# wvu-navLab/corenav-GP

Measured on AMD Instinct MI355X. Metric: GP-fits/s, higher is better.
Workload: dtype f64; 1 GPU; BASELINE configs[1]: batch of independent fixed-theta GP fits, N=2048 d=6 M=599 kernel=SE-ARD f64; streams=0, pipeline_depth=1, N=2048, d=6, M=599, inputs=resident in HBM, ranks=1

## Files before the change

corenav_gp_amd/csrc/cgp_kernels_fused.hpp:

```cpp
#pragma once
#include "cgp_kernels.hpp"

namespace cgp {

#ifndef CGP_SKIP_DEAD_WAVE
#define CGP_SKIP_DEAD_WAVE 1
#endif
constexpr bool kSkipDeadWave = CGP_SKIP_DEAD_WAVE != 0;

template <typename T>
__device__ __forceinline__ void stage_first_chunk(const T *gR, size_t ldR, const T *gC, size_t ldC, T *smem, int tid) {
  constexpr int CH = KT * LDST;
  if constexpr (sizeof(T) == 8) {
    typedef __attribute__((address_space(3))) void lds_void;
    typedef const __attribute__((address_space(1))) void gbl_void;
    const int lane = tid & 63;
    const int wave = __builtin_amdgcn_readfirstlane(tid >> 6);
#pragma unroll
    for (int i = 0; i < KT / 4; ++i) {
      const int col = wave * (KT / 4) + i;
      __builtin_amdgcn_global_load_lds((gbl_void *)(gR + (size_t)col * ldR + lane * 2), (lds_void *)(smem + col * LDST), 16, 0, 0);
      __builtin_amdgcn_global_load_lds((gbl_void *)(gC + (size_t)col * ldC + lane * 2), (lds_void *)(smem + CH + col * LDST), 16, 0, 0);
    }
  } else {
// ... 365 lines not shown
constexpr int BXP_NBUF = 3;
struct BxPlaneSrc {
  const unsigned short *gR, *gC;
  size_t chunk_stride, plane_stride;
  __device__ __forceinline__ void init(const unsigned short *planes, size_t plane_elems, int ld, int chunk0, int row_tile, int col_tile, int tid) {
    const int lane = tid & 63, wave = __builtin_amdgcn_readfirstlane(tid >> 6);
    const int slot = 32 * wave + (lane >> 1);
    const int h = ((lane & 1) ^ (slot >> 2) ^ (slot >> 4)) & 1;
    const int rowR = (slot & ~31) | ((slot & 15) << 1) | ((slot >> 4) & 1);
    chunk_stride = (size_t)ld * BXS;
    plane_stride = plane_elems;
    const unsigned short *base = planes + (size_t)chunk0 * chunk_stride;
    gR = base + ((size_t)row_tile * TS + rowR) * BXS + 8 * h;
    gC = base + ((size_t)col_tile * TS + slot) * BXS + 8 * h;
  }
  __device__ __forceinline__ void issue(int c, unsigned char *smem_bytes, int buf, int wave) const {
    typedef __attribute__((address_space(3))) void lds_void;
    typedef const __attribute__((address_space(1))) void gbl_void;
    const unsigned short *r = gR + (size_t)c * chunk_stride, *q = gC + (size_t)c * chunk_stride;
    unsigned char *dst = smem_bytes + buf + wave * 1024;
#pragma unroll
    for (int pl = 0; pl < 3; ++pl) {
      __builtin_amdgcn_global_load_lds((gbl_void *)(r + pl * plane_stride), (lds_void *)(dst + pl * 2 * BX_PLANE), 16, 0, 0);
      __builtin_amdgcn_global_load_lds((gbl_void *)(q + pl * plane_stride), (lds_void *)(dst + (3 + pl) * 2 * BX_PLANE), 16, 0, 0);
    }
  }
};
__device__ __forceinline__ void store_tile_planes(const Prec<float>::acc_t (&acc)[NCB][2], unsigned short *planes, size_t plane_elems, int ld, int rt, int k,
                                                  int tid) {
  const int lane = tid & 63, l15 = lane & 15, lq = lane >> 4;
  const int wave = __builtin_amdgcn_readfirstlane(tid >> 6);
  typedef unsigned bxu2 __attribute__((ext_vector_type(2)));
  unsigned short *out = planes + ((size_t)(k * (TS / KT)) * ld + (size_t)rt * TS + wave * 32 + 2 * l15) * BXS + 4 * lq;
#pragma unroll
  for (int cb = 0; cb < NCB; ++cb) {
    const float v[8] = {acc[cb][0][0], acc[cb][0][1], acc[cb][0][2], acc[cb][0][3], acc[cb][1][0], acc[cb][1][1], acc[cb][1][2], acc[cb][1][3]};
    bxu4 w[3];
    bx_split8(v, w);
    unsigned short *o = out + (size_t)cb * ld * BXS;
#pragma unroll
    for (int pl = 0; pl < 3; ++pl) {
      *reinterpret_cast<bxu2 *>(o + pl * plane_elems) = bxu2{w[pl][0], w[pl][1]};
      *reinterpret_cast<bxu2 *>(o + pl * plane_elems + BXS) = bxu2{w[pl][2], w[pl][3]};
    }
  }
}
__device__ __forceinline__ void bx6p_loop(Prec<float>::acc_t (&acc)[NCB][2], const BxPlaneSrc &src, int nchunk, float *smem, int tid, const float *zs, float *ms,
                                          bool live, const float *gR32, size_t ldR32) {
  if (nchunk <= 0) return;
  unsigned char *sb = reinterpret_cast<unsigned char *>(smem);
  const int lane = tid & 63, l15 = lane & 15, lq = lane >> 4;
  const int wave = __builtin_amdgcn_readfirstlane(tid >> 6);
  const int hi = lq >> 1;
  const unsigned base = (unsigned)(size_t)smem;
  const unsigned lb0[2] = {base + 2 * bx_pos(wave * 32 + l15, lq & 1), base + 2 * bx_pos(wave * 32 + DB + l15, lq & 1)};
  const unsigned la0[2] = {base + 2 * (3 * BX_PLANE + bx_pos(l15, lq & 1)), base + 2 * (3 * BX_PLANE + bx_pos(DB + l15, lq & 1) - DB * BXS)};
  int buf = 0;
  for (int c = 0; c < nchunk; ++c) {
    asm volatile("s_waitcnt vmcnt(6)" ::: "memory");
    lds_barrier();
    const int nb = buf == 0 ? 2 * BXP_BUF : buf - BXP_BUF;
    src.issue(c + 2 < nchunk ? c + 2 : nchunk - 1, sb, nb, wave);
    if (live) {
      const unsigned la[2] = {la0[0] + buf, la0[1] + buf}, lb[2] = {lb0[0] + buf, lb0[1] + buf};
      bx6_compute_pipe<0>(acc, la, lb, hi);
    }
    buf = buf == 2 * BXP_BUF ? 0 : buf + BXP_BUF;
  }
  asm volatile("s_waitcnt vmcnt(0)" ::: "memory");
  __syncthreads();
  if (zs) {
    const int r = tid & (TS - 1), h8 = 8 * (tid >> 7), zfirst = nchunk - TS / KT;
    float pz = 0.f, pv = 0.f;
    const float *g = gR32 + (size_t)(zfirst * KT + h8) * ldR32 + r;
#pragma unroll
    for (int c = 0; c < TS / KT; ++c) {
      float x[8];
#pragma unroll
      for (int i = 0; i < 8; ++i) x[i] = g[(size_t)(c * KT + i) * ldR32];
#pragma unroll
      for (int i = 0; i < 8; ++i) {
        pz = __builtin_fmaf(x[i], zs[c * KT + h8 + i], pz);
        pv = __builtin_fmaf(x[i], x[i], pv);
      }
    }
    smem[tid] = pz;
    smem[2 * TS + tid] = pv;
    __syncthreads();
    if (lane < 16) {
#pragma unroll
      for (int j = 0; j < 2; ++j) {
        const int rr = wave * 32 + 2 * lane + j;
        ms[j] = smem[rr] + smem[TS + rr];
        ms[2 + j] = smem[2 * TS + rr] + smem[3 * TS + rr];
      }
    }
    __syncthreads();
  }
}

template <typename T, int R = 4> struct RowFrag {
  using vec2 = T __attribute__((ext_vector_type(2)));
  vec2 r[R][KT / 4];
};
#ifndef CGP_MID_RING
#define CGP_MID_RING 4
#endif
template <typename T, bool MID> constexpr int deep_ring() { return (MID && sizeof(T) == 4) ? CGP_MID_RING : 4; }
template <int R> constexpr int deep_dist() { return R == 4 ? 2 : 5; }

template <typename T, int SLOT, int R>
__device__ __forceinline__ void rfrag_load(RowFrag<T, R> &f, const T *gRl, size_t ldR, int chunk, int lq) {
#pragma unroll
  for (int ks = 0; ks < KT / 4; ++ks) {
    const T *src = gRl + (size_t)(chunk * KT + ks * 4 + lq) * ldR;
    if constexpr (sizeof(T) == 8) asm volatile("global_load_dwordx4 %0, %1, off" : "=&v"(f.r[SLOT][ks]) : "v"(src));
    else asm volatile("global_load_dwordx2 %0, %1, off" : "=&v"(f.r[SLOT][ks]) : "v"(src));
  }
}

template <typename T> constexpr int cpanel_loads() { return sizeof(T) == 8 ? KT / 4 : KT / 2; }
template <typename T>
__device__ __forceinline__ void cpanel_stage(const T *gC, size_t ldC, int chunk, T *buf, int lane, int wave) {
  typedef __attribute__((address_space(3))) void lds_void;
  typedef const __attribute__((address_space(1))) void gbl_void;
#pragma unroll
  for (int i = 0; i < KT / 4; ++i) {
    const int col = wave * (KT / 4) + i;
    const T *src = gC + (size_t)(chunk * KT + col) * ldC;
    if constexpr (sizeof(T) == 8) {
      __builtin_amdgcn_global_load_lds((gbl_void *)(src + lane * 2), (lds_void *)(buf + col * LDST), 16, 0, 0);
    } else {
      __builtin_amdgcn_global_load_lds((gbl_void *)(src + lane), (lds_void *)(buf + col * LDST), 4, 0, 0);
      __builtin_amdgcn_global_load_lds((gbl_void *)(src + 64 + lane), (lds_void *)(buf + col * LDST + 64), 4, 0, 0);
    }
  }
}

template <typename T, int R = 4>
__device__ __forceinline__ void rdirect_prologue(RowFrag<T, R> &f, const T *gR, size_t ldR, const T *gC, size_t ldC,
                                                 int nchunk, T *smem, int tid) {
  constexpr int CH = KT * LDST;
  if (nchunk <= 0) return;
  const int lane = tid & 63;
  const int wave = __builtin_amdgcn_readfirstlane(tid >> 6);
  const T *gRl = gR + wave * 32 + 2 * (lane & 15);
  static_for<0, deep_dist<R>()>([&](auto jc) {
    constexpr int J = decltype(jc)::value;
    cpanel_stage<T>(gC, ldC, J, smem + J * CH, lane, wave);
    rfrag_load<T, J>(f, gRl, ldR, J, lane >> 4);
  });
}

template <typename T, int R, int S, bool ISSUE, int WAITN, bool ACC = false>
__device__ __forceinline__ void rdirect_step(typename Prec<T>::acc_t (&acc)[NCB][2], RowFrag<T, R> &f, const T *gRl, size_t ldR,
                                             const T *gC, size_t ldC, int c, T *smem, int lane, int wave,
                                             const T *zs = nullptr, T *ms = nullptr) {
  using P = Prec<T>;
  constexpr int CH = KT * LDST;
  constexpr int D = deep_dist<R>();
  const int l15 = lane & 15, lq = lane >> 4;
  static_assert(WAITN >= 0 && WAITN <= 63, "vmcnt is a 6-bit counter");
  asm volatile("s_waitcnt vmcnt(%0)\n\ts_barrier" ::"n"(WAITN) : "memory");
#pragma unroll
  for (int ks = 0; ks < KT / 4; ++ks) asm volatile("" : "+v"(f.r[S][ks]));
  if constexpr (ISSUE) {
    cpanel_stage<T>(gC, ldC, c + D, smem + ((S + D) % R) * CH, lane, wave);
    rfrag_load<T, (S + D) % R>(f, gRl, ldR, c + D, lq);
  }
  const T *cur = smem + S * CH + lq * LDST + l15;
  T fa[2][NCB];
#pragma unroll
  for (int cb = 0; cb < NCB; ++cb) fa[0][cb] = cur[cb * DB];
#pragma unroll
  for (int ks = 0; ks < KT / 4; ++ks) {
    if (ks + 1 < KT / 4) {
#pragma unroll
      for (int cb = 0; cb < NCB; ++cb) fa[(ks + 1) & 1][cb] = cur[(ks + 1) * 4 * LDST + cb * DB];
    }
    const typename RowFrag<T, R>::vec2 fb = f.r[S][ks];
    if constexpr (ACC) {
      const T zv = zs[ks * 4 + lq];
      ms[0] = __builtin_fma(fb[0], zv, ms[0]);
      ms[1] = __builtin_fma(fb[1], zv, ms[1]);
      ms[2] = __builtin_fma(fb[0], fb[0], ms[2]);
      ms[3] = __builtin_fma(fb[1], fb[1], ms[3]);
    }
#pragma unroll
    for (int cb = 0; cb < NCB; ++cb) {
      acc[cb][0] = P::mfma(fa[ks & 1][cb], fb[0], acc[cb][0]);
      acc[cb][1] = P::mfma(fa[ks & 1][cb], fb[1], acc[cb][1]);
    }
  }
}

template <typename T, int R = 4>
__device__ __forceinline__ void mfma_rowpanel_loop_rdirect(typename Prec<T>::acc_t (&acc)[NCB][2], RowFrag<T, R> &f, const T *gR,
                                                           size_t ldR, const T *gC, size_t ldC, int nchunk, T *smem, int tid,
                                                           const T *zs, T (&ms)[4]) {
  if (nchunk <= 0) return;
  constexpr int D = deep_dist<R>();
  constexpr int L = cpanel_loads<T>() + KT / 4;
  static_assert((D - 1) * L <= 63 && D < R && 8 % R == 0, "ring / distance / vmcnt");
  const int lane = tid & 63;
  const int wave = __builtin_amdgcn_readfirstlane(tid >> 6);
  const T *gRl = gR + wave * 32 + 2 * (lane & 15);
  int c = 0;
  for (; c + 8 < nchunk; c += R) {
    static_for<0, R>([&](auto jc) {
      constexpr int J = decltype(jc)::value;
      rdirect_step<T, R, J, true, (D - 1) * L>(acc, f, gRl, ldR, gC, ldC, c + J, smem, lane, wave);
    });
  }
  static_for<0, 8>([&](auto jc) {
    constexpr int J = decltype(jc)::value;
    constexpr int behind = (D - 1) < (7 - J) ? (D - 1) : (7 - J);
    rdirect_step<T, R, J % R, (J + D < 8), behind * L, true>(acc, f, gRl, ldR, gC, ldC, c + J, smem, lane, wave, zs + J * KT, ms);
  });
}

constexpr int TRI_PD = 2;
__device__ __forceinline__ constexpr int tri_buf(int i) { return i * KT * LDST; }

template <typename T> constexpr int tri_dma_loads() { return sizeof(T) == 8 ? KT / 4 : KT / 2; }
template <typename T, bool DEEP = sizeof(T) == 8>
__device__ __forceinline__ void stage_chunk_tri(const T *gR, size_t ldR, int chunk, T *buf, int tid) {
  if constexpr (DEEP) {
    typedef __attribute__((address_space(3))) void lds_void;
    typedef const __attribute__((address_space(1))) void gbl_void;
    const int lane = tid & 63;
    const int wave = __builtin_amdgcn_readfirstlane(tid >> 6);
#pragma unroll
    for (int i = 0; i < KT / 4; ++i) {
      const int col = wave * (KT / 4) + i;
      const T *src = gR + (size_t)(chunk * KT + col) * ldR;
      if constexpr (sizeof(T) == 8) {
        __builtin_amdgcn_global_load_lds((gbl_void *)(src + lane * 2), (lds_void *)(buf + col * LDST), 16, 0, 0);
      } else {
        __builtin_amdgcn_global_load_lds((gbl_void *)(src + lane), (lds_void *)(buf + col * LDST), 4, 0, 0);
        __builtin_amdgcn_global_load_lds((gbl_void *)(src + 64 + lane), (lds_void *)(buf + col * LDST + 64), 4, 0, 0);
      }
    }
  } else {
    using vec8 = T __attribute__((ext_vector_type(8)));
    const int sc = tid >> 4, sr = (tid & 15) * 8;
    *reinterpret_cast<vec8 *>(buf + sc * LDST + sr) = *reinterpret_cast<const vec8 *>(gR + sr + (size_t)(chunk * KT + sc) * ldR);
  }
}

template <typename T, int W, bool DEEP>
__device__ __forceinline__ void syrk_tri_wave(typename Prec<T>::acc_t (&acc)[NCB][2], const T *gR, size_t ldR, int nchunk,
                                              T *smem, int tid) {
  using P = Prec<T>;
  constexpr int RB0 = W, RB1 = NCB - 1 - W;
  const int lane = tid & 63;
  const int l15 = lane & 15, lq = lane >> 4;

  auto compute = [&](const T *cur) {
#pragma unroll
    for (int ks = 0; ks < KT / 4; ++ks) {
      const T *ra = cur + (ks * 4 + lq) * LDST + l15;
      T fa[RB1 + 1];
#pragma unroll
      for (int cb = 0; cb <= RB1; ++cb) fa[cb] = ra[cb * DB];
#pragma unroll
      for (int cb = 0; cb <= RB1; ++cb) {
        if (cb <= RB0) acc[cb][0] = P::mfma(fa[cb], fa[RB0], acc[cb][0]);
        acc[cb][1] = P::mfma(fa[cb], fa[RB1], acc[cb][1]);
      }
    }
  };

  if constexpr (DEEP) {
    for (int c = 0; c < nchunk; ++c) {
      if (c + 1 < nchunk) {
        if constexpr (sizeof(T) == 8) asm volatile("s_waitcnt vmcnt(4)\n\ts_barrier" ::: "memory");
        else asm volatile("s_waitcnt vmcnt(8)\n\ts_barrier" ::: "memory");
      } else asm volatile("s_waitcnt vmcnt(0)\n\ts_barrier" ::: "memory");
      static_assert(tri_dma_loads<double>() == 4 && tri_dma_loads<float>() == 8, "vmcnt constants");
      if (c + TRI_PD < nchunk) stage_chunk_tri<T, true>(gR, ldR, c + TRI_PD, smem + tri_buf((c + TRI_PD) % (TRI_PD + 1)), tid);
      compute(smem + tri_buf(c % (TRI_PD + 1)));
    }
  } else {
    using vec8 = T __attribute__((ext_vector_type(8)));
    const int sc = tid >> 4, sr = (tid & 15) * 8;
    const T *src = gR + sr + (size_t)sc * ldR;
    __syncthreads();
    for (int c = 0; c < nchunk; ++c) {
      vec8 pr;
      if (c + 1 < nchunk) pr = *reinterpret_cast<const vec8 *>(src + (size_t)((c + 1) * KT) * ldR);
      compute(smem + tri_buf(c & 1));
      if (c + 1 < nchunk) *reinterpret_cast<vec8 *>(smem + tri_buf((c + 1) & 1) + sc * LDST + sr) = pr;
      __syncthreads();
    }
  }
}

template <typename T, bool DEEP = sizeof(T) == 8>
__device__ __forceinline__ void mfma_syrk_tri_loop(typename Prec<T>::acc_t (&acc)[NCB][2], const T *gR, size_t ldR,
                                                   int nchunk, T *smem, int tid) {
  const int wave = __builtin_amdgcn_readfirstlane(tid >> 6);
  switch (wave) {
    case 0: syrk_tri_wave<T, 0, DEEP>(acc, gR, ldR, nchunk, smem, tid); break;
    case 1: syrk_tri_wave<T, 1, DEEP>(acc, gR, ldR, nchunk, smem, tid); break;
    case 2: syrk_tri_wave<T, 2, DEEP>(acc, gR, ldR, nchunk, smem, tid); break;
    default: syrk_tri_wave<T, 3, DEEP>(acc, gR, ldR, nchunk, smem, tid); break;
  }
}
template <typename T, bool DEEP = sizeof(T) == 8>
__device__ __forceinline__ void tri_prologue(const T *gR, size_t ldR, int nchunk, T *smem, int tid) {
  if (nchunk > 0) stage_chunk_tri<T, DEEP>(gR, ldR, 0, smem + tri_buf(0), tid);
  if (DEEP && nchunk > 1) stage_chunk_tri<T, DEEP>(gR, ldR, 1, smem + tri_buf(1), tid);
}

constexpr int BXT_FLOATS = 3 * BX_PLANE / 2;
template <int D> struct BxTriStage {
  __amdgpu_buffer_rsrc_t rR;
  int ldR4, vR, offR;
  float xr[D][8];
  __device__ __forceinline__ void init(const float *gR, size_t ldR, int nchunk, int tid) {
    const int r = tid & (TS - 1), h = tid >> 7;
    rR = __builtin_amdgcn_make_buffer_rsrc(const_cast<float *>(gR), 0, (int)(((size_t)(nchunk > 0 ? nchunk : 0) * KT * ldR) * sizeof(float)), 0x00020000);
    ldR4 = (int)ldR * 4;
    vR = 4 * r + 8 * h * ldR4;
    offR = bx_pos(r, h);
  }
  template <int S> __device__ __forceinline__ void load(int chunk) {
#pragma unroll
    for (int i = 0; i < 8; ++i) xr[S][i] = __builtin_bit_cast(float, __builtin_amdgcn_raw_buffer_load_b32(rR, vR, (chunk * KT + i) * ldR4, 0));
  }
  template <int S> __device__ __forceinline__ void store(float *planes) { bx_split_store(xr[S], reinterpret_cast<unsigned short *>(planes), offR); }
};
template <int D> __device__ __forceinline__ void bx6_tri_prologue(BxTriStage<D> &st) {
  static_assert(D == 2 || D == 4, "register sets (the plane buffer of a chunk follows the parity of its set)");
  st.template load<0>(0);
  st.template load<1>(1);
  if (D > 2) st.template load<2 % D>(2);
  if (D > 2) st.template load<3 % D>(3);
}
template <int W, int BO>
__device__ __forceinline__ void bx6_tri_compute(Prec<float>::acc_t (&acc)[NCB][2], const unsigned (&e)[2], bool hi) {
  constexpr int RB0 = W, RB1 = NCB - 1 - W, PB = 2 * BX_PLANE, CBB = 2 * DB * BXS;
  const unsigned o02 = hi ? 2 * PB : 0, o01 = hi ? PB : 0, o20 = hi ? 0 : 2 * PB, o10 = hi ? 0 : PB;
  bxu4 a02[RB1 + 1], a01[RB1 + 1];
  bxu4 b20[2] = {bx_rd(e[RB0 & 1] + o20, BO + RB0 * CBB), bx_rd(e[RB1 & 1] + o20, BO + RB1 * CBB)};
  static_for<0, RB1 + 1>([&](auto cc) {
    constexpr int CB = decltype(cc)::value;
    a02[CB] = bx_rd(e[CB & 1] + o02, BO + CB * CBB);
  });
  bxu4 b10[2] = {bx_rd(e[RB0 & 1] + o10, BO + RB0 * CBB), bx_rd(e[RB1 & 1] + o10, BO + RB1 * CBB)};
  asm volatile("s_waitcnt lgkmcnt(2)" : "+v"(b20[0]), "+v"(b20[1]));
  static_for<0, RB1 + 1>([&](auto cc) { bx_tie(a02[decltype(cc)::value]); });
  static_for<0, RB1 + 1>([&](auto cc) {
    constexpr int CB = decltype(cc)::value;
    a01[CB] = bx_rd(e[CB & 1] + o01, BO + CB * CBB);
  });
  const bf8 c20[2] = {__builtin_bit_cast(bf8, b20[0]), __builtin_bit_cast(bf8, b20[1])};
  static_for<0, RB1 + 1>([&](auto cc) {
    constexpr int CB = decltype(cc)::value;
    const bf8 a = __builtin_bit_cast(bf8, a02[CB]);
    if constexpr (CB <= RB0) acc[CB][0] = __builtin_amdgcn_mfma_f32_16x16x32_bf16(a, c20[0], acc[CB][0], 0, 0, 0);
    acc[CB][1] = __builtin_amdgcn_mfma_f32_16x16x32_bf16(a, c20[1], acc[CB][1], 0, 0, 0);
  });
  asm volatile("s_waitcnt lgkmcnt(0)" : "+v"(b10[0]), "+v"(b10[1]));
  static_for<0, RB1 + 1>([&](auto cc) { bx_tie(a01[decltype(cc)::value]); });
  const bf8 c10[2] = {__builtin_bit_cast(bf8, b10[0]), __builtin_bit_cast(bf8, b10[1])};
  const bf8 c01[2] = {__builtin_bit_cast(bf8, a01[RB0]), __builtin_bit_cast(bf8, a01[RB1])};
  static_for<0, RB1 + 1>([&](auto cc) {
    constexpr int CB = decltype(cc)::value;
    const bf8 a = __builtin_bit_cast(bf8, a01[CB]);
// ... 387 lines not shown
  if (tid == 0 && bad != 0 && p.info[b] == 0) p.info[b] = bad;
  for (int idx = tid; idx < 28 * DB * DB; idx += 256) {
    const int blk = idx >> 8, e = idx & 255;
    int i = 1, rem = blk;
    while (rem >= i) {
      rem -= i;
      ++i;
    }
    const int j = rem, c = e >> 4, r = e & 15;
    Wk[wimg_blk(i, j) + c * DB + r] = -Bk[tri_blk(i, j) + r * DB + c];
  }
}

enum { DIAG_FULL = 0, DIAG_PARTIAL = 1, DIAG_FINISH = 2 };
__device__ __forceinline__ int img_slots(const FitArgs &p) { return p.img_slots > 0 ? p.img_slots : 2; }
constexpr bool kTriDiag = true;
constexpr int DPART = 2 * NCB * 4 * 256;

template <typename T, bool TRI, bool STORE>
__device__ __forceinline__ void acc_image(typename Prec<T>::acc_t (&acc)[NCB][2], T *__restrict__ img, int tid) {
  const int wave = __builtin_amdgcn_readfirstlane(tid >> 6);
#pragma unroll
  for (int cb = 0; cb < NCB; ++cb)
#pragma unroll
    for (int j = 0; j < 2; ++j) {
      if (TRI && cb > (j ? NCB - 1 - wave : wave)) continue;
#pragma unroll
      for (int r = 0; r < 4; ++r) {
        T *q = img + ((cb * 2 + j) * 4 + r) * 256 + tid;
        if constexpr (STORE) *q = acc[cb][j][r];
        else acc[cb][j][r] = *q;
      }
    }
}

template <typename T> constexpr int potf2_lds_elems() { return TS * LDP + 8 * DB * DB + 4 * DB * DB + 8; }
template <typename T, int MODE, bool TRI, bool DEEP = sizeof(T) == 8, bool FAT = false, bool MAT = false>
__device__ __forceinline__ void diag_next(const FitArgs &p, typename Prec<T>::acc_t (&acc)[NCB][2], T *__restrict__ smem,
                                          T *__restrict__ Lw, int b, int kn, int tid, PhaseClock *pc = nullptr, bool img_ready = false) {
  using P = Prec<T>;
  using vec2 = T __attribute__((ext_vector_type(2)));
  const int ld = p.ld;
  const int lane = tid & 63;
  const int wave = __builtin_amdgcn_readfirstlane(tid >> 6);
  const int l15 = lane & 15;
  constexpr int CH2 = 2 * KT * LDST;
  if constexpr (MODE == DIAG_FINISH) {
    __builtin_amdgcn_fence(__ATOMIC_RELEASE, "workgroup");
    __syncthreads();
    __builtin_amdgcn_fence(__ATOMIC_ACQUIRE, "workgroup");
  }
  const bool from_image = MODE == DIAG_FINISH && kn >= 3;
  const int c_first = from_image ? (kn - 2) * (TS / KT) : 0;
  const int c_last = (MODE == DIAG_PARTIAL ? kn - 2 : kn) * (TS / KT);
  const int nchunk = c_last - c_first;
  const T *gR = Lw + (size_t)kn * TS + (size_t)c_first * KT * ld;
  T *img = reinterpret_cast<T *>(p.dpart) + ((size_t)b * img_slots(p) + kn % img_slots(p)) * DPART;
  constexpr bool BXT = kF32Bf16x6 && kBxTri && sizeof(T) == 4 && TRI && DEEP;
  BxTriStage<kBxMidSets> bxt;
  {
    GramPre<T> gp;
    if (!from_image) gram_prefetch<T>(p, b, kn, kn, tid, gp);
    if constexpr (BXT) {
      bxt.init(gR, (size_t)ld, nchunk, tid);
      bx6_tri_prologue(bxt);
    } else if constexpr (TRI) tri_prologue<T, DEEP>(gR, (size_t)ld, nchunk, smem, tid);
    else if (nchunk > 0) stage_first_chunk<T>(gR, (size_t)ld, gR, (size_t)ld, smem, tid);
    if (from_image) {
      if (!img_ready) acc_image<T, TRI, false>(acc, img, tid);
    } else gram_apply<T, TRI, 2, MAT>(p, acc, smem + (BXT ? BXT_FLOATS : CH2), b, kn, kn, tid, gp);
  }
  if (pc) pc->lap(p, 344);
  if constexpr (BXT) bx6_syrk_tri_loop(acc, bxt, nchunk, smem, tid);
  else if constexpr (TRI) mfma_syrk_tri_loop<T, DEEP>(acc, gR, (size_t)ld, nchunk, smem, tid);
  else mfma_rowpanel_loop<T, true>(acc, gR, (size_t)ld, gR, (size_t)ld, nchunk, smem, tid);
  if (pc) pc->lap(p, 345);
  if constexpr (MODE == DIAG_PARTIAL) {
    acc_image<T, TRI, true>(acc, img, tid);
    return;
  }
  __syncthreads();
  T *tile = Lw + (size_t)(kn * TS) * ld + (size_t)kn * TS;
  if constexpr (FAT) {
    static_assert(!FAT || TRI, "the fat form takes the triangular accumulator layout");
    T *At = smem;
    T *Dv = At + TS * LDP;
    T *Ts = Dv + 8 * DB * DB;
    int *flag = reinterpret_cast<int *>(Ts + 4 * DB * DB);
#pragma unroll
    for (int cb = 0; cb < NCB; ++cb)
#pragma unroll
      for (int j = 0; j < 2; ++j) {
        const int rb = j ? NCB - 1 - wave : wave;
        if (cb <= rb) {
#pragma unroll
          for (int r = 0; r < 4; ++r) At[(cb * DB + P::drow(lane, r)) * LDP + rb * DB + l15] = -acc[cb][j][r];
        }
      }
    if (tid == 0) *flag = 0;
    __syncthreads();
    if (pc) pc->lap(p, 346);
    potf2_tile<T>(p, At, Dv, Ts, flag, tile, ld, b, kn, tid);
    if (pc) {
      pc->lap(p, 347);
      pc->count(p, 351);
    }
    return;
  }
  if constexpr (TRI) {
#pragma unroll
    for (int cb = 0; cb < NCB; ++cb)
#pragma unroll
      for (int j = 0; j < 2; ++j) {
        const int rb = j ? NCB - 1 - wave : wave;
        if (cb <= rb) {
#pragma unroll
          for (int r = 0; r < 4; ++r) smem[tri_blk(rb, cb) + P::drow(lane, r) * DB + l15] = -acc[cb][j][r];
        }
      }
  } else {
    const int rb = 2 * wave + (l15 >> 3), rin = (2 * l15) & 15;
#pragma unroll
    for (int cb = 0; cb < NCB; ++cb)
      if (cb <= rb) {
#pragma unroll
        for (int r = 0; r < 4; ++r) {
          vec2 v;
          v[0] = -acc[cb][0][r];
          v[1] = -acc[cb][1][r];
          *reinterpret_cast<vec2 *>(smem + tri_blk(rb, cb) + P::drow(lane, r) * DB + rin) = v;
        }
      }
  }
  __syncthreads();
  T *Wk = reinterpret_cast<T *>(p.Winv) + (size_t)b * p.winv_stride + (size_t)kn * WIMG;
  if (pc) pc->lap(p, 346);
  diag_factor_packed<T>(p, smem, tile, ld, Wk, b, kn, tid);
  if (pc) {
    pc->lap(p, 347);
    pc->count(p, 351);
  }
}

template <typename T, bool FAT = false, bool MAT = false>
__global__ __launch_bounds__(256, 2) void k_diag_lean(FitArgs p, int k) {
  extern __shared__ __attribute__((aligned(16))) char smem_raw[];
  T *smem = reinterpret_cast<T *>(smem_raw);
  const int b = blockIdx.x;
  T *Lw = reinterpret_cast<T *>(p.Lw) + (size_t)b * p.lw_stride;
  typename Prec<T>::acc_t acc[NCB][2];
  diag_next<T, DIAG_FULL, kTriDiag, sizeof(T) == 8 || FAT, FAT, MAT>(p, acc, smem, Lw, b, k, threadIdx.x);
}

template <typename T>
__device__ __forceinline__ void trmm_in_registers(const FitArgs &p, typename Prec<T>::acc_t (&acc)[NCB][2], T *__restrict__ smem,
                                                  int b, int k, int tid, PhaseClock *pc = nullptr, int wslot = 0, bool live = true) {
  using P = Prec<T>;
  using acc_t = typename P::acc_t;
  const int lane = tid & 63, l15 = lane & 15;
  const T *__restrict__ Wk = reinterpret_cast<const T *>(p.Winv) + (size_t)b * p.winv_stride + (size_t)k * WIMG;
  {
    typedef __attribute__((address_space(3))) void lds_void;
    typedef const __attribute__((address_space(1))) void gbl_void;
    const int wave = __builtin_amdgcn_readfirstlane(tid >> 6);
    constexpr int PER = 1024 / (int)sizeof(T);
    constexpr int NI = WIMG / PER / 4;
    static_assert(WIMG % (4 * PER) == 0, "image is a whole number of 4 KiB rounds");
#pragma unroll
    for (int i = 0; i < NI; ++i) {
      const int off = (i * 4 + wave) * PER;
      __builtin_amdgcn_global_load_lds((gbl_void *)(Wk + off + lane * (16 / (int)sizeof(T))), (lds_void *)(smem + off), 16, 0, 0);
    }
    asm volatile("s_waitcnt vmcnt(0)" ::: "memory");
  }
  __syncthreads();
  if (pc) pc->lap(p, wslot);
  if (!live) return;

#pragma unroll
  for (int cb = NCB - 1; cb >= 0; --cb) {
    acc_t t0 = acc_t{0, 0, 0, 0}, t1 = t0;
    const T *wrow = smem + (cb * (cb + 1) / 2) * DB * DB + l15;
#pragma unroll
    for (int qb = 0; qb <= cb; ++qb) {
#pragma unroll
      for (int r = 0; r < 4; ++r) {
        const T a = wrow[qb * DB * DB + P::drow(lane, r) * DB];
        t0 = P::mfma(a, acc[qb][0][r], t0);
        t1 = P::mfma(a, acc[qb][1][r], t1);
      }
    }
    acc[cb][0] = t0;
    acc[cb][1] = t1;
    __builtin_amdgcn_sched_barrier(0);
  }
}

__device__ __forceinline__ void trmm_bx6_operand(int round, int ci, int &m, int &cb) {
  if (round) { m = 0; cb = ci; }
  else if (ci < 2) { m = 3; cb = 6 + ci; }
  else if (ci < 6) { m = 2; cb = 2 + ci; }
  else { m = 1; cb = ci - 4; }
}
template <int M, int CI0>
__device__ __forceinline__ void trmm_bx6_pair(Prec<float>::acc_t (&acc)[NCB][2], const unsigned short *planes, int lane) {
  using acc_t = Prec<float>::acc_t;
  bf8 bp[2][3];
#pragma unroll
  for (int j = 0; j < 2; ++j) {
    const float v[8] = {acc[2 * M][j][0], acc[2 * M][j][1], acc[2 * M][j][2], acc[2 * M][j][3],
                        acc[2 * M + 1][j][0], acc[2 * M + 1][j][1], acc[2 * M + 1][j][2], acc[2 * M + 1][j][3]};
    bxu4 w[3];
    bx_split8(v, w);
#pragma unroll
    for (int pl = 0; pl < 3; ++pl) bp[j][pl] = __builtin_bit_cast(bf8, w[pl]);
    acc[2 * M][j] = acc_t{0, 0, 0, 0};
    acc[2 * M + 1][j] = acc_t{0, 0, 0, 0};
  }
  static_for<0, (NCB - 2 * M) / 2>([&](auto hc) {
    constexpr int H = decltype(hc)::value, CB = 2 * M + 2 * H, CI = CI0 + 2 * H;
    bf8 ap[2][3];
#pragma unroll
    for (int u = 0; u < 2; ++u)
#pragma unroll
      for (int pl = 0; pl < 3; ++pl) ap[u][pl] = bx_ld8(planes + (((CI + u) * 3 + pl) * 64 + lane) * 8);
    constexpr int NT8 = 8;
    constexpr int TA[NT8] = {1, 2, 0, 2, 1, 0, 1, 0}, TB[NT8] = {2, 1, 2, 0, 1, 1, 0, 0};
#pragma unroll
    for (int t = 0; t < NT8; ++t)
#pragma unroll
      for (int u = 0; u < 2; ++u)
#pragma unroll
        for (int j = 0; j < 2; ++j)
          acc[CB + u][j] = __builtin_amdgcn_mfma_f32_16x16x32_bf16(ap[u][TA[t]], bp[j][TB[t]], acc[CB + u][j], 0, 0, 0);
  });
}
__device__ __forceinline__ void trmm_bx6(const FitArgs &p, Prec<float>::acc_t (&acc)[NCB][2], float *__restrict__ smem, int b, int k, int tid,
                                         PhaseClock *pc, int wslot, bool live) {
  const int lane = tid & 63, c = lane & 15, g = lane >> 4;
  const float *__restrict__ Wk = reinterpret_cast<const float *>(p.Winv) + (size_t)b * p.winv_stride + (size_t)k * WIMG;
  unsigned short *planes = reinterpret_cast<unsigned short *>(smem);
#pragma unroll
  for (int round = 0; round < 2; ++round) {
    constexpr int NOPW[2] = {3, 2};
    const int wv = __builtin_amdgcn_readfirstlane(tid >> 6);
    float v[3][8];
#pragma unroll
    for (int i = 0; i < 3; ++i) {
      if (i >= NOPW[round]) continue;
      int m, cb;
      trmm_bx6_operand(round, wv + 4 * i, m, cb);
      const float *w0 = Wk + (cb * (cb + 1) / 2 + 2 * m) * DB * DB + (4 * g) * DB + c;
      const bool second = 2 * m + 1 <= cb;
#pragma unroll
      for (int r = 0; r < 4; ++r) {
        v[i][r] = w0[r * DB];
        v[i][4 + r] = second ? w0[DB * DB + r * DB] : 0.f;
      }
    }
#pragma unroll
    for (int i = 0; i < 3; ++i) {
      if (i >= NOPW[round]) continue;
      bxu4 w[3];
      bx_split8(v[i], w);
#pragma unroll
      for (int pl = 0; pl < 3; ++pl) *reinterpret_cast<bxu4 *>(planes + (((wv + 4 * i) * 3 + pl) * 64 + lane) * 8) = w[pl];
    }
    __syncthreads();
    if (pc && round == 0) pc->lap(p, wslot);
    if (live) {
      if (round == 0) {
        trmm_bx6_pair<3, 0>(acc, planes, lane);
        trmm_bx6_pair<2, 2>(acc, planes, lane);
        trmm_bx6_pair<1, 6>(acc, planes, lane);
      } else trmm_bx6_pair<0, 0>(acc, planes, lane);
    }
    if (round == 0) __syncthreads();
  }
}

template <typename T>
__device__ __forceinline__ void store_tile(const typename Prec<T>::acc_t (&acc)[NCB][2], T *__restrict__ tile, int ld, int tid) {
  using P = Prec<T>;
  using vec2 = T __attribute__((ext_vector_type(2)));
  const int lane = tid & 63, l15 = lane & 15;
  const int wave = __builtin_amdgcn_readfirstlane(tid >> 6);
  T *__restrict__ out = tile + wave * 32 + 2 * l15;
#pragma unroll
  for (int cb = 0; cb < NCB; ++cb)
#pragma unroll
    for (int r = 0; r < 4; ++r) {
      vec2 v;
      v[0] = acc[cb][0][r];
      v[1] = acc[cb][1][r];
      *reinterpret_cast<vec2 *>(out + (size_t)(cb * DB + P::drow(lane, r)) * ld) = v;
    }
}
template <typename T, bool ADD>
__device__ __forceinline__ void load_tile(typename Prec<T>::acc_t (&acc)[NCB][2], const T *tile, int ld, int tid) {
  using P = Prec<T>;
  using vec2 = T __attribute__((ext_vector_type(2)));
  const int lane = tid & 63, l15 = lane & 15;
  const int wave = __builtin_amdgcn_readfirstlane(tid >> 6);
  const T *src = tile + wave * 32 + 2 * l15;
#pragma unroll
  for (int cb = 0; cb < NCB; ++cb)
#pragma unroll
    for (int r = 0; r < 4; ++r) {
      const vec2 v = *reinterpret_cast<const vec2 *>(src + (size_t)(cb * DB + P::drow(lane, r)) * ld);
      acc[cb][0][r] = ADD ? acc[cb][0][r] + v[0] : v[0];
      acc[cb][1][r] = ADD ? acc[cb][1][r] + v[1] : v[1];
    }
}


template <typename T, bool DEEP, bool MAT = false>
__device__ __forceinline__ void panel_partial(const FitArgs &p, typename Prec<T>::acc_t (&acc)[NCB][2], T *__restrict__ smem, int b,
                                              int k, int tid) {
  constexpr int CH2 = 2 * KT * LDST;
  const int kc = k + 1, rt = k + 2, ld = p.ld, nchunk = k * (TS / KT);
  const T *Lw = reinterpret_cast<const T *>(p.Lw) + (size_t)b * p.lw_stride;
  const T *gR = Lw + (size_t)rt * TS, *gC = Lw + (size_t)kc * TS;
  GramPre<T> gp;
  gram_prefetch<T>(p, b, kc, rt, tid, gp);
  if constexpr (DEEP) {
    constexpr int R = deep_ring<T, true>();
    RowFrag<T, R> rf;
    T *zs = smem + R * KT * LDST;
    if (tid < TS) zs[tid] = T(0);
    T ms[4] = {T(0), T(0), T(0), T(0)};
    rdirect_prologue<T, R>(rf, gR, (size_t)ld, gC, (size_t)ld, nchunk, smem, tid);
    gram_apply<T, false, 2, MAT>(p, acc, smem + (R - 2) * KT * LDST, b, kc, rt, tid, gp);
    mfma_rowpanel_loop_rdirect<T, R>(acc, rf, gR, (size_t)ld, gC, (size_t)ld, nchunk, smem, tid, zs, ms);
  } else {
    if (nchunk > 0) stage_first_chunk<T>(gR, (size_t)ld, gC, (size_t)ld, smem, tid);
    gram_apply<T, false, 2, MAT>(p, acc, smem + CH2, b, kc, rt, tid, gp);
    mfma_rowpanel_loop<T, true>(acc, gR, (size_t)ld, gC, (size_t)ld, nchunk, smem, tid);
  }
  acc_image<T, false, true>(acc, reinterpret_cast<T *>(p.pimg) + ((size_t)b * img_slots(p) + kc % img_slots(p)) * DPART, tid);
}

#ifndef CGP_IMG_EARLY
#define CGP_IMG_EARLY 1
#endif
template <typename T, bool MID> constexpr bool mid_fat() { return MID && sizeof(T) == 4; }
template <typename T, bool DIAGNEXT, bool DEEP, bool MID, bool MAT = false>
__device__ __forceinline__ void panel_tile_body(const FitArgs &p, int k, int b, int rt, int c_first, bool finish_next, bool from_image,
                                                T *smem, int tid) {
  using P = Prec<T>;
  using acc_t = typename P::acc_t;
  acc_t acc[NCB][2];
  T *Lw = reinterpret_cast<T *>(p.Lw) + (size_t)b * p.lw_stride;
  const int ld = p.ld;
  PhaseClock pc;
  pc.start(p, tid);
  const int ps = finish_next ? 336 : 64 + 8 * (k & 31);

  constexpr int CH2 = 2 * KT * LDST;
  const T *gR = Lw + (size_t)rt * TS + (size_t)(c_first * KT) * ld, *gC = Lw + (size_t)k * TS + (size_t)(c_first * KT) * ld;
  if (CGP_DBG_ON(p, 4096)) gR = reinterpret_cast<const T *>(p.Lw) + (size_t)(b & 7) * p.lw_stride + (size_t)p.NT * TS;
  if (CGP_DBG_ON(p, 8192)) gC = reinterpret_cast<const T *>(p.Lw) + (size_t)(b & 7) * p.lw_stride + (size_t)k * TS;
  const int nchunk = k * (TS / KT) - c_first;
  const T *pimg = reinterpret_cast<const T *>(p.pimg) + ((size_t)b * img_slots(p) + k % img_slots(p)) * DPART;
  const bool accm = p.macc != nullptr && rt >= p.NT && k > 0;
  const bool live = !(kSkipDeadWave && !DEEP && sizeof(T) == 4 && rt >= p.NT && !p.xid &&
                      (rt - p.NT) * TS + __builtin_amdgcn_readfirstlane(tid >> 6) * 32 > p.M);
  constexpr int R = DEEP ? deep_ring<T, MID>() : 4;
  constexpr bool BX6 = kF32Bf16x6 && sizeof(T) == 4 && (!DEEP || MID);
  constexpr bool BXDBL = DEEP;
  constexpr int BXD = DEEP ? kBxMidSets : 1;
  constexpr bool PL = kMidPlanes && BX6 && MID;
  constexpr int GRAM_OFF = PL ? 2 * BXP_BUF / 4 : (BX6 ? BX_FLOATS : CH2);
  T *zs = smem + (PL ? BXP_NBUF * BXP_BUF / 4 : (BX6 ? bx_z_offset<BXDBL>() : R * KT * LDST));
  if (tid < TS) zs[tid] = accm ? Lw[(size_t)((k - 1) * TS + tid) * ld + (size_t)p.NT * TS + p.M] : T(0);
  T ms[4] = {T(0), T(0), T(0), T(0)};
  if constexpr (DEEP && !BX6) {
    RowFrag<T, R> rf;
    {
      GramPre<T> gp;
      if (!(MID && from_image)) gram_prefetch<T>(p, b, k, rt, tid, gp);
      rdirect_prologue<T, R>(rf, gR, (size_t)ld, gC, (size_t)ld, nchunk, smem, tid);
      if (MID && from_image) acc_image<T, false, false>(acc, const_cast<T *>(pimg), tid);
      else gram_apply<T, false, 2, MAT>(p, acc, smem + (R - 2) * KT * LDST, b, k, rt, tid, gp, &pc, ps + 6);
    }
    pc.lap(p, ps + 0);
    mfma_rowpanel_loop_rdirect<T, R>(acc, rf, gR, (size_t)ld, gC, (size_t)ld, nchunk, smem, tid, zs, ms);
  } else {
    BxStage<PL ? 1 : BXD> bxs;
    BxPlaneSrc bps;
    {
      GramPre<T> gp;
      if (!(MID && from_image)) gram_prefetch<T>(p, b, k, rt, tid, gp);
      if (nchunk > 0) {
        if constexpr (PL) {
          bps.init(reinterpret_cast<const unsigned short *>(p.Lp) + (size_t)b * p.lp_stride, p.lp_stride / 3, ld, c_first, rt, k, tid);
          const int wv = __builtin_amdgcn_readfirstlane(tid >> 6);
          bps.issue(0, reinterpret_cast<unsigned char *>(smem), 0, wv);
          bps.issue(1, reinterpret_cast<unsigned char *>(smem), BXP_BUF, wv);
        } else if constexpr (BX6) {
          bxs.init(gR, (size_t)ld, gC, (size_t)ld, nchunk, tid);
          bx6_prologue(bxs, nchunk);
        } else stage_first_chunk<T>(gR, (size_t)ld, gC, (size_t)ld, smem, tid);
      }
      if (CGP_DBG_ON(p, 16384)) {
#pragma unroll
        for (int cb = 0; cb < NCB; ++cb)
#pragma unroll
          for (int j = 0; j < 2; ++j)
#pragma unroll
            for (int r = 0; r < 4; ++r) acc[cb][j][r] = gp.v[0];
      } else if (MID && from_image) acc_image<T, false, false>(acc, const_cast<T *>(pimg), tid);
      else gram_apply<T, false, 2, MAT>(p, acc, smem + GRAM_OFF, b, k, rt, tid, gp, &pc, ps + 6, -1, live);
    }
    pc.lap(p, ps + 0);
    if constexpr (PL) bx6p_loop(acc, bps, nchunk, smem, tid, accm ? zs : nullptr, ms, live, gR, (size_t)ld);
    else if constexpr (BX6) bx6_loop<BXD, BXDBL>(acc, bxs, nchunk, smem, tid, accm ? zs : nullptr, ms, live);
    else mfma_rowpanel_loop<T, true>(acc, gR, (size_t)ld, gC, (size_t)ld, nchunk, smem, tid, accm ? zs : nullptr, ms, live);
  }
  pc.lap(p, ps + 1);
  if (accm) {
#pragma unroll
    for (int q = 0; q < 4; ++q) {
      ms[q] += __shfl_xor(ms[q], 16);
      ms[q] += __shfl_xor(ms[q], 32);
    }
    const int lane = tid & 63;
    const int wave = __builtin_amdgcn_readfirstlane(tid >> 6);
    if (lane < 16) {
#pragma unroll
      for (int j = 0; j < 2; ++j) {
        const int m = (rt - p.NT) * TS + wave * 32 + 2 * lane + j;
        if (m < p.M) {
          double *pm = p.macc + (size_t)b * p.M + m, *pv = p.vacc + (size_t)b * p.M + m;
          const double om = k == 1 ? 0.0 : __hip_atomic_load(pm, __ATOMIC_RELAXED, __HIP_MEMORY_SCOPE_AGENT);
          const double ov = k == 1 ? 0.0 : __hip_atomic_load(pv, __ATOMIC_RELAXED, __HIP_MEMORY_SCOPE_AGENT);
          __hip_atomic_store(pm, om + (double)ms[j], __ATOMIC_RELAXED, __HIP_MEMORY_SCOPE_AGENT);
          __hip_atomic_store(pv, ov + (double)ms[2 + j], __ATOMIC_RELAXED, __HIP_MEMORY_SCOPE_AGENT);
        }
      }
    }
  }
  __syncthreads();
  pc.lap(p, ps + 2);
  if (!CGP_DBG_ON(p, 64)) {
    if constexpr (kF32Bf16x6 && kBxTrmm && sizeof(T) == 4) trmm_bx6(p, acc, smem, b, k, tid, &pc, ps + 3, live);
    else trmm_in_registers<T>(p, acc, smem, b, k, tid, &pc, ps + 3, live);
  }
  pc.lap(p, ps + 4);
  if (live && (!CGP_DBG_ON(p, 32768) || acc[0][0][0] == T(12345.678)))
  store_tile<T>(acc, Lw + (size_t)(k * TS) * ld + (size_t)rt * TS, ld, tid);
  if constexpr (PL) {
    if (live) store_tile_planes(acc, reinterpret_cast<unsigned short *>(p.Lp) + (size_t)b * p.lp_stride, p.lp_stride / 3, ld, rt, k, tid);
  }
  pc.lap(p, ps + 5);
  pc.count(p, ps + 7);
  if constexpr (DIAGNEXT) {
    if (finish_next) {
      bool img_ready = false;
      if constexpr (MID && CGP_IMG_EARLY) {
        if (k + 1 >= 3) {
          const T *img = reinterpret_cast<const T *>(p.dpart) + ((size_t)b * img_slots(p) + (k + 1) % img_slots(p)) * DPART;
          acc_image<T, kTriDiag, false>(acc, const_cast<T *>(img), tid);
          img_ready = true;
        }
      }
      diag_next<T, DIAG_FINISH, kTriDiag, DEEP, mid_fat<T, MID>(), MAT>(p, acc, smem, Lw, b, k + 1, tid, &pc, img_ready);
    }
  }
}

#ifndef CGP_KINDA_PRIO
#define CGP_KINDA_PRIO 0
#endif
#ifndef CGP_F32_FULL_OCC
#define CGP_F32_FULL_OCC 4
#endif
constexpr int F32_FULL_OCC = CGP_F32_FULL_OCC;
template <typename T, bool DIAGNEXT = false, bool DEEP = sizeof(T) == 8, bool MID = false, bool MAT = false>
__global__ __launch_bounds__(256, sizeof(T) == 4 ? (DEEP ? ((MID && (CGP_MID_RING > 4 || CGP_F32_BF16X6)) ? 2 : 3) : F32_FULL_OCC) : 2) void k_panel(FitArgs p, int k) {
  using P = Prec<T>;
  using acc_t = typename P::acc_t;
  extern __shared__ __attribute__((aligned(16))) char smem_raw[];
  T *smem = reinterpret_cast<T *>(smem_raw);
  const int tid = threadIdx.x;
  int bt, b, rt;
  int c_first = 0;
  bool finish_next = false, from_image = false;
  acc_t acc[NCB][2];
  SpanClock sc;
  sc.enter(p, k, tid);
  if constexpr (DIAGNEXT) {
    const int Tg = gridDim.x, B = gridDim.y;
    const int lin = blockIdx.y * Tg + blockIdx.x;
    const int nA = (p.diag_slots & 1) ? B : 0, nB = (p.diag_slots & 2) ? B : 0, nC = (MID && (p.diag_slots & 4)) ? B : 0;
    int ia = -1, io = lin;
    const int stride = p.diag_stride, ablk = nA >> 8, oblk = (Tg * B - nA) >> 8;
    if (nA > 0 && (B & 255) == 0 && stride > 0 && (ablk - 1) * stride < ablk + oblk) {
      const int j = lin >> 8, r = lin & 255;
      const int before = min((j + stride - 1) / stride, ablk);
      if (j % stride == 0 && j / stride < ablk) ia = (j / stride) * 256 + r;
      else io = (j - before) * 256 + r;
    } else if (lin < nA) ia = lin;
    else io = lin - nA;
    if (CGP_DBG_ON(p, 65536) && (ia >= 0 || io < nB)) {
      if (ia < 0) return;
    }
    if (ia >= 0) {
      b = ia;
      rt = k + 1;
      finish_next = !CGP_DBG_ON(p, 65536);
      if constexpr (MID && CGP_KINDA_PRIO > 0) __builtin_amdgcn_s_setprio(CGP_KINDA_PRIO);
      if (MID && (p.diag_slots & 8)) {
        from_image = true;
        c_first = (k - 1) * (TS / KT);
      }
    } else if (io < nB) {
      b = io;
      T *LwB = reinterpret_cast<T *>(p.Lw) + (size_t)b * p.lw_stride;
      diag_next<T, DIAG_PARTIAL, kTriDiag, DEEP, false, MAT>(p, acc, smem, LwB, b, k + 2, tid);
      sc.leave(p, k, tid);
      return;
    } else if (MID && io < nB + nC) {
      panel_partial<T, DEEP, MAT>(p, acc, smem, io - nB, k, tid);
      sc.leave(p, k, tid);
      return;
    } else {
      const int l2 = io - nB - nC, To = Tg - (nA ? 1 : 0) - (nB ? 1 : 0) - (nC ? 1 : 0);
      if ((B & 7) == 0) {
        const int xcd = l2 & 7, slot = l2 >> 3;
        bt = slot % To;
        b = (slot / To) * 8 + xcd;
      } else {
        bt = l2 % To;
        b = l2 / To;
      }
      const int first = k + 1 + (nA ? 1 : 0);
      const int nin = p.NT - first > 0 ? p.NT - first : 0;
      rt = bt < nin ? first + bt : p.NT + (bt - nin);
    }
  } else {
    tile_fit_of_block(bt, b);
    rt = row_tile_of(bt + p.tile_off, k + 1, p.NT, p.rows_from_extra);
  }
  panel_tile_body<T, DIAGNEXT, DEEP, MID, MAT>(p, k, b, rt, c_first, finish_next, from_image, smem, tid);
  sc.leave(p, k, tid);
}

constexpr int HR = TS / 2;
template <typename T, int SLOT>
__device__ __forceinline__ void r16_load(T (&f)[4][KT / 4], const T *gRl, size_t ldR, int chunk, int lq) {
#pragma unroll
  for (int ks = 0; ks < KT / 4; ++ks) {
    const T *src = gRl + (size_t)(chunk * KT + ks * 4 + lq) * ldR;
    if constexpr (sizeof(T) == 8) asm volatile("global_load_dwordx2 %0, %1, off" : "=&v"(f[SLOT][ks]) : "v"(src));
    else asm volatile("global_load_dword %0, %1, off" : "=&v"(f[SLOT][ks]) : "v"(src));
  }
}
template <typename T, int S, bool ISSUE, int WAITN, bool ACC>
__device__ __forceinline__ void r16_step(typename Prec<T>::acc_t (&acc)[NCB][1], T (&f)[4][KT / 4], const T *gRl, size_t ldR, const T *gC,
                                         size_t ldC, int c, T *smem, int lane, int wave, const T *zs, T *ms) {
  using P = Prec<T>;
  constexpr int CH = KT * LDST;
  const int l15 = lane & 15, lq = lane >> 4;
  asm volatile("s_waitcnt vmcnt(%0)\n\ts_barrier" ::"n"(WAITN) : "memory");
#pragma unroll
  for (int ks = 0; ks < KT / 4; ++ks) asm volatile("" : "+v"(f[S][ks]));
  if constexpr (ISSUE) {
    cpanel_stage<T>(gC, ldC, c + 2, smem + ((S + 2) & 3) * CH, lane, wave);
    r16_load<T, (S + 2) & 3>(f, gRl, ldR, c + 2, lq);
  }
  const T *cur = smem + S * CH + lq * LDST + l15;
  T fa[2][NCB];
#pragma unroll
  for (int cb = 0; cb < NCB; ++cb) fa[0][cb] = cur[cb * DB];
#pragma unroll
  for (int ks = 0; ks < KT / 4; ++ks) {
    if (ks + 1 < KT / 4) {
#pragma unroll
      for (int cb = 0; cb < NCB; ++cb) fa[(ks + 1) & 1][cb] = cur[(ks + 1) * 4 * LDST + cb * DB];
    }
    const T fb = f[S][ks];
    if constexpr (ACC) {
      const T zv = zs[ks * 4 + lq];
      ms[0] = __builtin_fma(fb, zv, ms[0]);
      ms[1] = __builtin_fma(fb, fb, ms[1]);
    }
#pragma unroll
    for (int cb = 0; cb < NCB; ++cb) acc[cb][0] = P::mfma(fa[ks & 1][cb], fb, acc[cb][0]);
  }
}

template <typename T, bool MAT = false>
__global__ __launch_bounds__(256, sizeof(T) == 4 ? 4 : 2) void k_rows64(FitArgs p, int k) {
  using P = Prec<T>;
  using acc_t = typename P::acc_t;
  extern __shared__ __attribute__((aligned(16))) char smem_raw[];
  T *smem = reinterpret_cast<T *>(smem_raw);
  const int tid = threadIdx.x, lane = tid & 63, l15 = lane & 15, lq = lane >> 4;
  const int wave = __builtin_amdgcn_readfirstlane(tid >> 6);
  int h, b;
// ... 680 lines not shown
```

Before: 11280 fits/s.

## Prefetch W_k triangle image into freed ring slots during the rowpanel tail

Starts the global-to-LDS loads of the inverse-diagonal W_k image while the last steps of the f64 rowpanel MFMA loop are still running, placing pieces into ring slots once they are no longer needed. The image is stored in reversed block order so the first slots freed hold the blocks the TRMM needs first. The TRMM then waits only for the remaining pieces, and the last pieces are waited on partway through the block loop. The aim is to hide W_k load latency behind the GEMM tail. The cost is tighter vmcnt accounting and extra barriers, with a risk of LDS hazards if the slot-lifetime assumptions are wrong.

```diff
diff --git a/corenav_gp_amd/csrc/cgp_kernels_fused.hpp b/corenav_gp_amd/csrc/cgp_kernels_fused.hpp
--- a/corenav_gp_amd/csrc/cgp_kernels_fused.hpp
+++ b/corenav_gp_amd/csrc/cgp_kernels_fused.hpp
@@ -541,10 +541,26 @@
   });
 }
 
-template <typename T, int R, int S, bool ISSUE, int WAITN, bool ACC = false>
+constexpr int WBLK = NCB * (NCB + 1) / 2;
+constexpr int wimg_cum(int slots) { return slots <= 0 ? 0 : (slots * 18) / 4; }
+template <typename T, int I0, int I1>
+__device__ __forceinline__ void wimg_stage_rev(const T *__restrict__ Wk, T *__restrict__ smem, int lane, int wave) {
+  typedef __attribute__((address_space(3))) void lds_void;
+  typedef const __attribute__((address_space(1))) void gbl_void;
+  constexpr int PER = 1024 / (int)sizeof(T), PPB = DB * DB / PER;
+  static_assert(sizeof(T) == 8 && WIMG == 4 * KT * LDST && WIMG / PER == 4 * 18 && I0 >= 0 && I1 <= 18, "image = chunk ring");
+#pragma unroll
+  for (int i = I0; i < I1; ++i) {
+    const int piece = i * 4 + wave;
+    const T *src = Wk + ((WBLK - 1 - piece / PPB) * PPB + piece % PPB) * PER + lane * (16 / (int)sizeof(T));
+    __builtin_amdgcn_global_load_lds((gbl_void *)src, (lds_void *)(smem + piece * PER), 16, 0, 0);
+  }
+}
+
+template <typename T, int R, int S, bool ISSUE, int WAITN, bool ACC = false, int WI0 = 0, int WI1 = 0>
 __device__ __forceinline__ void rdirect_step(typename Prec<T>::acc_t (&acc)[NCB][2], RowFrag<T, R> &f, const T *gRl, size_t ldR,
                                              const T *gC, size_t ldC, int c, T *smem, int lane, int wave,
-                                             const T *zs = nullptr, T *ms = nullptr) {
+                                             const T *zs = nullptr, T *ms = nullptr, const T *Wk = nullptr) {
   using P = Prec<T>;
   constexpr int CH = KT * LDST;
   constexpr int D = deep_dist<R>();
@@ -557,6 +573,7 @@
     cpanel_stage<T>(gC, ldC, c + D, smem + ((S + D) % R) * CH, lane, wave);
     rfrag_load<T, (S + D) % R>(f, gRl, ldR, c + D, lq);
   }
+  if constexpr (WI1 > WI0) wimg_stage_rev<T, WI0, WI1>(Wk, smem, lane, wave);
   const T *cur = smem + S * CH + lq * LDST + l15;
   T fa[2][NCB];
 #pragma unroll
@@ -583,14 +600,15 @@
   }
 }
 
-template <typename T, int R = 4>
+template <typename T, int R = 4, bool WPRE = false>
 __device__ __forceinline__ void mfma_rowpanel_loop_rdirect(typename Prec<T>::acc_t (&acc)[NCB][2], RowFrag<T, R> &f, const T *gR,
                                                            size_t ldR, const T *gC, size_t ldC, int nchunk, T *smem, int tid,
-                                                           const T *zs, T (&ms)[4]) {
+                                                           const T *zs, T (&ms)[4], const T *Wk = nullptr) {
   if (nchunk <= 0) return;
   constexpr int D = deep_dist<R>();
   constexpr int L = cpanel_loads<T>() + KT / 4;
   static_assert((D - 1) * L <= 63 && D < R && 8 % R == 0, "ring / distance / vmcnt");
+  static_assert(!WPRE || (R == 4 && D == 2 && sizeof(T) == 8), "W_k under the tail: slot s is free from tail step s + 5 on");
   const int lane = tid & 63;
   const int wave = __builtin_amdgcn_readfirstlane(tid >> 6);
   const T *gRl = gR + wave * 32 + 2 * (lane & 15);
@@ -604,7 +622,10 @@
   static_for<0, 8>([&](auto jc) {
     constexpr int J = decltype(jc)::value;
     constexpr int behind = (D - 1) < (7 - J) ? (D - 1) : (7 - J);
-    rdirect_step<T, R, J % R, (J + D < 8), behind * L, true>(acc, f, gRl, ldR, gC, ldC, c + J, smem, lane, wave, zs + J * KT, ms);
+    constexpr int W0 = WPRE ? wimg_cum(J - 5) : 0, W1 = WPRE ? wimg_cum(J - 4) : 0;
+    static_assert(behind * L + W0 <= 63, "vmcnt");
+    rdirect_step<T, R, J % R, (J + D < 8), behind * L + W0, true, W0, W1>(acc, f, gRl, ldR, gC, ldC, c + J, smem, lane, wave, zs + J * KT,
+                                                                          ms, Wk);
   });
 }
 
@@ -1298,14 +1319,22 @@
   diag_next<T, DIAG_FULL, kTriDiag, sizeof(T) == 8 || FAT, FAT, MAT>(p, acc, smem, Lw, b, k, threadIdx.x);
 }
 
-template <typename T>
+template <typename T, bool REV = false>
 __device__ __forceinline__ void trmm_in_registers(const FitArgs &p, typename Prec<T>::acc_t (&acc)[NCB][2], T *__restrict__ smem,
-                                                  int b, int k, int tid, PhaseClock *pc = nullptr, int wslot = 0, bool live = true) {
+                                                  int b, int k, int tid, PhaseClock *pc = nullptr, int wslot = 0, bool live = true,
+                                                  bool under_loop = false) {
   using P = Prec<T>;
   using acc_t = typename P::acc_t;
   const int lane = tid & 63, l15 = lane & 15;
   const T *__restrict__ Wk = reinterpret_cast<const T *>(p.Winv) + (size_t)b * p.winv_stride + (size_t)k * WIMG;
-  {
+  if constexpr (REV) {
+    const int wave = __builtin_amdgcn_readfirstlane(tid >> 6);
+    if (!under_loop) {
+      wimg_stage_rev<T, 0, wimg_cum(3)>(Wk, smem, lane, wave);
+      asm volatile("s_waitcnt vmcnt(0)\n\ts_barrier" ::: "memory");
+    }
+    wimg_stage_rev<T, wimg_cum(3), wimg_cum(4)>(Wk, smem, lane, wave);
+  } else {
     typedef __attribute__((address_space(3))) void lds_void;
     typedef const __attribute__((address_space(1))) void gbl_void;
     const int wave = __builtin_amdgcn_readfirstlane(tid >> 6);
@@ -1318,20 +1347,24 @@
       __builtin_amdgcn_global_load_lds((gbl_void *)(Wk + off + lane * (16 / (int)sizeof(T))), (lds_void *)(smem + off), 16, 0, 0);
     }
     asm volatile("s_waitcnt vmcnt(0)" ::: "memory");
-  }
-  __syncthreads();
+    __syncthreads();
+  }
   if (pc) pc->lap(p, wslot);
   if (!live) return;
 
 #pragma unroll
   for (int cb = NCB - 1; cb >= 0; --cb) {
+    if constexpr (REV) {
+      if (cb == 3) asm volatile("s_waitcnt vmcnt(0)\n\ts_barrier" ::: "memory");
+    }
     acc_t t0 = acc_t{0, 0, 0, 0}, t1 = t0;
-    const T *wrow = smem + (cb * (cb + 1) / 2) * DB * DB + l15;
+    const T *wrow = REV ? smem + (WBLK - 1 - cb * (cb + 1) / 2) * DB * DB + l15 : smem + (cb * (cb + 1) / 2) * DB * DB + l15;
+    constexpr int QST = REV ? -DB * DB : DB * DB;
 #pragma unroll
     for (int qb = 0; qb <= cb; ++qb) {
 #pragma unroll
       for (int r = 0; r < 4; ++r) {
-        const T a = wrow[qb * DB * DB + P::drow(lane, r) * DB];
+        const T a = wrow[qb * QST + P::drow(lane, r) * DB];
         t0 = P::mfma(a, acc[qb][0][r], t0);
         t1 = P::mfma(a, acc[qb][1][r], t1);
       }
@@ -1514,6 +1547,7 @@
   constexpr int R = DEEP ? deep_ring<T, MID>() : 4;
   constexpr bool BX6 = kF32Bf16x6 && sizeof(T) == 4 && (!DEEP || MID);
   constexpr bool BXDBL = DEEP;
+  constexpr bool WPRE = DEEP && sizeof(T) == 8;
   constexpr int BXD = DEEP ? kBxMidSets : 1;
   constexpr bool PL = kMidPlanes && BX6 && MID;
   constexpr int GRAM_OFF = PL ? 2 * BXP_BUF / 4 : (BX6 ? BX_FLOATS : CH2);
@@ -1530,7 +1564,8 @@
       else gram_apply<T, false, 2, MAT>(p, acc, smem + (R - 2) * KT * LDST, b, k, rt, tid, gp, &pc, ps + 6);
     }
     pc.lap(p, ps + 0);
-    mfma_rowpanel_loop_rdirect<T, R>(acc, rf, gR, (size_t)ld, gC, (size_t)ld, nchunk, smem, tid, zs, ms);
+    mfma_rowpanel_loop_rdirect<T, R, WPRE>(acc, rf, gR, (size_t)ld, gC, (size_t)ld, nchunk, smem, tid, zs, ms,
+                                           reinterpret_cast<const T *>(p.Winv) + (size_t)b * p.winv_stride + (size_t)k * WIMG);
   } else {
     BxStage<PL ? 1 : BXD> bxs;
     BxPlaneSrc bps;
@@ -1590,8 +1625,8 @@
   pc.lap(p, ps + 2);
   if (!CGP_DBG_ON(p, 64)) {
     if constexpr (kF32Bf16x6 && kBxTrmm && sizeof(T) == 4) trmm_bx6(p, acc, smem, b, k, tid, &pc, ps + 3, live);
-    else trmm_in_registers<T>(p, acc, smem, b, k, tid, &pc, ps + 3, live);
-  }
+    else trmm_in_registers<T, WPRE>(p, acc, smem, b, k, tid, &pc, ps + 3, live, nchunk > 0);
+  } else if constexpr (WPRE) asm volatile("s_waitcnt vmcnt(0)" ::: "memory");
   pc.lap(p, ps + 4);
   if (live && (!CGP_DBG_ON(p, 32768) || acc[0][0][0] == T(12345.678)))
   store_tile<T>(acc, Lw + (size_t)(k * TS) * ld + (size_t)rt * TS, ld, tid);
```

Result: no change. 11310 fits/s, median of 3 (+0.3%).
